# wp133716/test_isaacgym

Hardware: AMD Instinct MI355X
Metric: env-steps/sec (whole node), 4096 servo envs; 1/2/4/8-GPU scaling (higher is better)
Workload: dtype f32

## Files before the change

### test_isaacgym_amd/csrc/mg_rigid.hip

```cpp
#include "mg_internal.h"
#include "mg_math.h"
#include "mg_attractor.h"
#include "mg_contact.h"

#ifdef MG_RIGID1_STAMPS
#define MG_RIGID1_NSTAMP 18
__device__ unsigned long long g_rigid_stamp[4096][MG_RIGID1_NSTAMP];
extern "C" int mg_debug_rigid_stamps(unsigned long long* out, int nwaves) {
    if (nwaves > 4096) nwaves = 4096;
    return hipMemcpyFromSymbol(out, HIP_SYMBOL(g_rigid_stamp), (size_t)nwaves * MG_RIGID1_NSTAMP * 8) == hipSuccess
               ? 0
               : -1;
}
__device__ __forceinline__ unsigned long long rigid_stamp() {
    unsigned long long t;
    __builtin_amdgcn_sched_barrier(0);
    asm volatile("s_memtime %0\n\ts_waitcnt lgkmcnt(0)" : "=s"(t)::"memory");
    __builtin_amdgcn_sched_barrier(0);
    return t;
}
#define RSTAMP(k) do { const unsigned long long t_ = rigid_stamp(); \
    if (threadIdx.x == 0 && blockIdx.x < 4096) g_rigid_stamp[blockIdx.x][k] = t_; } while (0)
#define RUSE(v) asm volatile("" ::"v"(v))
#else
#define RSTAMP(k) do { } while (0)
#define RUSE(v) do { } while (0)
#endif

namespace {

__device__ __forceinline__ float fdot3(V3 a, V3 b, float acc) {
    return fmaf(a.z, b.z, fmaf(a.y, b.y, fmaf(a.x, b.x, acc)));
}
__device__ __forceinline__ V3 fmad3(V3 v, V3 d, float s) {
    return v3(fmaf(d.x, s, v.x), fmaf(d.y, s, v.y), fmaf(d.z, s, v.z));
}
struct BasisGen {
    static constexpr bool kPacked = false;
    V3 n, t1, t2;
    __device__ __forceinline__ float dn(V3 v) const { return vdot(n, v); }
    __device__ __forceinline__ float d1(V3 v) const { return vdot(t1, v); }
    __device__ __forceinline__ float d2(V3 v) const { return vdot(t2, v); }
    __device__ __forceinline__ V3 cn(V3 r) const { return vcross(r, n); }
    __device__ __forceinline__ V3 c1(V3 r) const { return vcross(r, t1); }
    __device__ __forceinline__ V3 c2(V3 r) const { return vcross(r, t2); }
    __device__ __forceinline__ V3 addn(V3 v, float s) const { return vmad(v, n, s); }
    __device__ __forceinline__ V3 add1(V3 v, float s) const { return vmad(v, t1, s); }
    __device__ __forceinline__ V3 add2(V3 v, float s) const { return vmad(v, t2, s); }
    __device__ __forceinline__ float vn(V3 v, V3 w, V3 r) const { return fdot3(w, cn(r), vdot(n, v)); }
    __device__ __forceinline__ float v1(V3 v, V3 w, V3 r) const { return fdot3(w, c1(r), vdot(t1, v)); }
    __device__ __forceinline__ float v2(V3 v, V3 w, V3 r) const { return fdot3(w, c2(r), vdot(t2, v)); }
    __device__ __forceinline__ float ps(float s0, V3 dx, V3 dth, V3 r) const {
        return fdot3(dth, cn(r), s0 + vdot(n, dx));
    }
    __device__ __forceinline__ V3 fn(V3 v, float dl, float invm) const { return fmad3(v, n, dl * invm); }
    __device__ __forceinline__ V3 f1(V3 v, float dl, float invm) const { return fmad3(v, t1, dl * invm); }
    __device__ __forceinline__ V3 f2(V3 v, float dl, float invm) const { return fmad3(v, t2, dl * invm); }
    __device__ __forceinline__ V3 iwn(const S3& I, V3 r) const { return symmul(I, cn(r)); }
    __device__ __forceinline__ V3 iw1(const S3& I, V3 r) const { return symmul(I, c1(r)); }
    __device__ __forceinline__ V3 iw2(const S3& I, V3 r) const { return symmul(I, c2(r)); }
    __device__ __forceinline__ float kn(V3 r, V3 In) const { return vdot(cn(r), In); }
    __device__ __forceinline__ float k1(V3 r, V3 I1) const { return vdot(c1(r), I1); }
    __device__ __forceinline__ float k2(V3 r, V3 I2) const { return vdot(c2(r), I2); }
};
struct BasisZ {
    static constexpr bool kPacked = true;
    __device__ __forceinline__ float dn(V3 v) const { return v.z; }
    __device__ __forceinline__ float d1(V3 v) const { return v.y; }
    __device__ __forceinline__ float d2(V3 v) const { return -v.x; }
    __device__ __forceinline__ V3 cn(V3 r) const { return v3(r.y, -r.x, 0.0f); }
    __device__ __forceinline__ V3 c1(V3 r) const { return v3(-r.z, 0.0f, r.x); }
    __device__ __forceinline__ V3 c2(V3 r) const { return v3(0.0f, -r.z, r.y); }
    __device__ __forceinline__ V3 addn(V3 v, float s) const { return v3(v.x, v.y, v.z + s); }
    __device__ __forceinline__ V3 add1(V3 v, float s) const { return v3(v.x, v.y + s, v.z); }
    __device__ __forceinline__ V3 add2(V3 v, float s) const { return v3(v.x - s, v.y, v.z); }
    __device__ __forceinline__ float vn(V3 v, V3 w, V3 r) const { return fmaf(w.y, -r.x, fmaf(w.x, r.y, v.z)); }
    __device__ __forceinline__ float v1(V3 v, V3 w, V3 r) const { return fmaf(w.z, r.x, fmaf(w.x, -r.z, v.y)); }
    __device__ __forceinline__ float v2(V3 v, V3 w, V3 r) const { return fmaf(w.z, r.y, fmaf(w.y, -r.z, -v.x)); }
    __device__ __forceinline__ float ps(float s0, V3 dx, V3 dth, V3 r) const {
        return fmaf(dth.y, -r.x, fmaf(dth.x, r.y, s0 + dx.z));
    }
    __device__ __forceinline__ V3 fn(V3 v, float dl, float invm) const { return v3(v.x, v.y, fmaf(dl, invm, v.z)); }
    __device__ __forceinline__ V3 f1(V3 v, float dl, float invm) const { return v3(v.x, fmaf(dl, invm, v.y), v.z); }
    __device__ __forceinline__ V3 f2(V3 v, float dl, float invm) const { return v3(fmaf(-dl, invm, v.x), v.y, v.z); }
    __device__ __forceinline__ V3 iwn(const S3& I, V3 r) const {
        const float a = r.y, b = -r.x;
        return v3(I.xx * a + I.xy * b, I.xy * a + I.yy * b, I.xz * a + I.yz * b);
    }
    __device__ __forceinline__ V3 iw1(const S3& I, V3 r) const {
        const float a = -r.z, c = r.x;
        return v3(I.xx * a + I.xz * c, I.xy * a + I.yz * c, I.xz * a + I.zz * c);
    }
    __device__ __forceinline__ V3 iw2(const S3& I, V3 r) const {
        const float b = -r.z, c = r.y;
        return v3(I.xy * b + I.xz * c, I.yy * b + I.yz * c, I.yz * b + I.zz * c);
    }
    __device__ __forceinline__ float kn(V3 r, V3 In) const { return r.y * In.x + -r.x * In.y; }
    __device__ __forceinline__ float k1(V3 r, V3 I1) const { return -r.z * I1.x + r.x * I1.z; }
    __device__ __forceinline__ float k2(V3 r, V3 I2) const { return -r.z * I2.y + r.y * I2.z; }
};

__device__ __forceinline__ float clamp_sym(float x, float lim) { return __builtin_amdgcn_fmed3f(x, -lim, lim); }

struct Slot {
    V3 r;
    float s0;
    float mu, e;
    float kn, kt1, kt2;
    float ln, lt1, lt2;
    float vn0;
    V3 In, I1, I2;
    bool on;
};

#define MG_OPAQUE3(v) asm volatile("" : "+v"((v).x), "+v"((v).y), "+v"((v).z))

template <bool CACHE, class B>
__device__ __forceinline__ void contact_normal(const B& G, Slot& c, V3& v, V3& w, float invm, const S3& Iw,
                                               float tgt) {
    if (!CACHE) MG_OPAQUE3(c.r);
    const float vn = G.vn(v, w, c.r);
    const float nl = fmaxf(fmaf(c.kn, tgt - vn, c.ln), 0.0f);
    const float dl = nl - c.ln;
    c.ln = nl;
    v = G.fn(v, dl, invm);
    w = fmad3(w, CACHE ? c.In : G.iwn(Iw, c.r), dl);
}

template <bool CACHE, class B>
__device__ __forceinline__ void contact_friction(const B& G, Slot& c, V3& v, V3& w, float invm, const S3& Iw) {
    if (!CACHE) MG_OPAQUE3(c.r);
    const float lim = c.mu * c.ln;
    const float vt1 = G.v1(v, w, c.r);
    const float n1 = clamp_sym(fmaf(-c.kt1, vt1, c.lt1), lim);
    const float d1 = n1 - c.lt1;
    c.lt1 = n1;
    v = G.f1(v, d1, invm);
    w = fmad3(w, CACHE ? c.I1 : G.iw1(Iw, c.r), d1);
    const float vt2 = G.v2(v, w, c.r);
    const float n2 = clamp_sym(fmaf(-c.kt2, vt2, c.lt2), lim);
    const float d2 = n2 - c.lt2;
    c.lt2 = n2;
    v = G.f2(v, d2, invm);
    w = fmad3(w, CACHE ? c.I2 : G.iw2(Iw, c.r), d2);
}

__device__ __forceinline__ float pos_target(const MgStep& P, float s) { return fminf(-s * P.inv_sub, P.max_depen); }
__device__ __forceinline__ float vel_target(const MgStep& P, float s, float e, float vn0) {
    float tgt = fminf(-s * P.inv_h, 0.0f);
    if (e > 0.0f && vn0 < -P.bounce_thresh) tgt = fmaxf(tgt, -e * vn0);
    return tgt;
}

__device__ __forceinline__ bool shape_pose_identity(const float* sh) {
    return sh[4] == 0.0f && sh[5] == 0.0f && sh[6] == 0.0f && sh[7] == 0.0f && sh[8] == 0.0f && sh[9] == 0.0f &&
           sh[10] == 1.0f;
}
__device__ __forceinline__ Q4 inertia_frame(Q4 q, Q4 iq) {
    if (iq.x == 0.0f && iq.y == 0.0f && iq.z == 0.0f && iq.w == 1.0f) return q;
    return qmul(q, iq);
}
__device__ __forceinline__ V3 com_world(V3 x, Q4 q, V3 com) {
    if (com.x == 0.0f && com.y == 0.0f && com.z == 0.0f) return x;
    return vadd(x, qrot(q, com));
}
__device__ __forceinline__ V3 origin_from_com(V3 xc, Q4 q, V3 com) {
    if (com.x == 0.0f && com.y == 0.0f && com.z == 0.0f) return xc;
    return vsub(xc, qrot(q, com));
}

template <bool BOX = false, class B, class F>
__device__ __forceinline__ void shape_candidates(const B& G, const MgStep& P, const float* sh, Q4 q, V3 x,
                                                 const float* hulls, F&& emit) {
    const int type = BOX ? MG_SHAPE_BOX : (int)sh[0];
    Q4 qs = q;
    V3 cs = x;
    if constexpr (!BOX) {
        if (!shape_pose_identity(sh)) {
            qs = qmul(q, q4(sh[7], sh[8], sh[9], sh[10]));
            cs = vadd(x, qrot(q, v3(sh[4], sh[5], sh[6])));
        }
    }
    const float mu = 0.5f * (sh[11] + P.mu_ground);
    const float e = 0.5f * (sh[12] + P.e_ground);
    if (type == MG_SHAPE_BOX) {
        const M3 Rs = qmat(qs);
        const float d0 = G.dn(Rs.c0), d1 = G.dn(Rs.c1), d2 = G.dn(Rs.c2);
        const float ad0 = fabsf(d0), ad1 = fabsf(d1), ad2 = fabsf(d2);
        int ia = 0;
        float best = ad0;
        if (ad1 > best) { ia = 1; best = ad1; }
        if (ad2 > best) ia = 2;
        const V3 a0 = vscale(Rs.c0, sh[1]);
        const V3 a1 = vscale(Rs.c1, sh[2]);
        const V3 a2 = vscale(Rs.c2, sh[3]);
        const float di = ia == 0 ? d0 : (ia == 1 ? d1 : d2);
        const V3 ai = ia == 0 ? a0 : (ia == 1 ? a1 : a2);
        const V3 e1 = ia == 0 ? a1 : a0;
        const V3 e2 = ia == 2 ? a1 : a2;
        const V3 u = vscale(ai, di > 0.0f ? -1.0f : 1.0f);
        const V3 cu = vadd(cs, u);
#pragma unroll
        for (int k = 0; k < 4; ++k) {
            const float sx = (k & 1) ? 1.0f : -1.0f;
            const float sy = (k & 2) ? 1.0f : -1.0f;
            const V3 p = vadd(vadd(cu, vscale(e1, sx)), vscale(e2, sy));
            emit(k, p, G.dn(p) + P.pd, mu, e);
        }
    } else if (type == MG_SHAPE_SPHERE) {
        const float rad = sh[1];
        emit(0, G.addn(cs, -rad), G.dn(cs) + P.pd - rad, mu, e);
    } else if (type == MG_SHAPE_CAPSULE) {
        const float rad = sh[1];
        const V3 ax = vscale(qrot(qs, v3(1.0f, 0.0f, 0.0f)), sh[2]);
#pragma unroll
        for (int k = 0; k < 2; ++k) {
            const V3 c = k ? vadd(cs, ax) : vsub(cs, ax);
            emit(k, G.addn(c, -rad), G.dn(c) + P.pd - rad, mu, e);
        }
    } else if (type == MG_SHAPE_CONVEX) {
        const float* hv = hulls + (int)sh[2];
        const int nv = (int)hv[0];
        float ks[4] = {0.0f, 0.0f, 0.0f, 0.0f};
        V3 kp[4];
        int kn = 0;
        for (int i = 0; i < nv; ++i) {
            const float* v = hv + MG_HULL_HEADER + 3 * i;
            const V3 p = vadd(cs, qrot(qs, v3(v[0], v[1], v[2])));
            const float sep = G.dn(p) + P.pd;
            if (!(sep < P.contact_offset)) continue;
            if (kn == 4 && !(sep < ks[3])) continue;
            int at = 0;
#pragma unroll
            for (int k = 0; k < 4; ++k)
                if (k < kn && ks[k] <= sep) at = k + 1;
#pragma unroll
            for (int k = 3; k > 0; --k)
                if (k > at) { ks[k] = ks[k - 1]; kp[k] = kp[k - 1]; }
#pragma unroll
            for (int k = 0; k < 4; ++k)
                if (k == at) { ks[k] = sep; kp[k] = p; }
            if (kn < 4) kn = kn + 1;
        }
#pragma unroll
        for (int k = 0; k < 4; ++k)
            if (k < kn) emit(k, kp[k], ks[k], mu, e);
    }
}

template <int MAXC, bool MULTI, bool ATTR, bool CREP, class B>
__device__ __forceinline__ void rigid_body(const B& G, const MgStep& P, const MgRigidArgs& A, int b) {
    constexpr bool CACHE = !MULTI;
    const int nb = A.nb;
    float* S = A.state;

    V3 x = v3(S[0 * nb + b], S[1 * nb + b], S[2 * nb + b]);
    Q4 q = q4(S[3 * nb + b], S[4 * nb + b], S[5 * nb + b], S[6 * nb + b]);
    V3 v = v3(S[7 * nb + b], S[8 * nb + b], S[9 * nb + b]);
    V3 w = v3(S[10 * nb + b], S[11 * nb + b], S[12 * nb + b]);

    const float* M = A.mass;
    const float invm = M[0 * nb + b];
    const V3 invI = v3(M[1 * nb + b], M[2 * nb + b], M[3 * nb + b]);
    const Q4 iq = q4(M[4 * nb + b], M[5 * nb + b], M[6 * nb + b], M[7 * nb + b]);
    const V3 com = v3(M[8 * nb + b], M[9 * nb + b], M[10 * nb + b]);

    const int tb = A.body_tmpl[b];
    const float lin_damp = A.tbf[tb * MG_TBODY_F_N + 0];
    const float ang_damp = A.tbf[tb * MG_TBODY_F_N + 1];
    const float max_lv = A.tbf[tb * MG_TBODY_F_N + 2];
    const float max_av = A.tbf[tb * MG_TBODY_F_N + 3];
    const float grav_on = A.tbf[tb * MG_TBODY_F_N + 4];
    const int sh0 = A.tbi[tb * MG_TBODY_I_N + 0];
    const int nsh = A.tbi[tb * MG_TBODY_I_N + 1];

    V3 fext = v3(0.0f, 0.0f, 0.0f), text = v3(0.0f, 0.0f, 0.0f);
    if (A.ext) {
        fext = v3(A.ext[0 * nb + b], A.ext[1 * nb + b], A.ext[2 * nb + b]);
        text = v3(A.ext[3 * nb + b], A.ext[4 * nb + b], A.ext[5 * nb + b]);
    }

    const float h = P.h;
    const float lin_keep = 1.0f - fminf(lin_damp * h, 1.0f);
    const float ang_keep = 1.0f - fminf(ang_damp * h, 1.0f);
    const float max_lv2 = max_lv * max_lv;
    const float max_av2 = max_av * max_av;
    const float* at = nullptr;
    if constexpr (ATTR) {
        const int ai = A.attr_idx[b];
        if (ai >= 0) at = A.attr + (size_t)ai * MG_ATTR_N;
    }

    q = qnormalize(q);
    V3 fsum = v3(0.0f, 0.0f, 0.0f);
    int crk = 0;

    for (int st = 0; st < P.substeps; ++st) {
        const S3 Iw = sym_rdrt(qmat(inertia_frame(q, iq)), invI);
        const V3 xc = com_world(x, q, com);

        if (grav_on != 0.0f) v = vmad(v, v3(P.g[0], P.g[1], P.g[2]), h);
        if (A.ext) {
            v = vmad(v, fext, invm * h);
            w = vmad(w, symmul(Iw, text), h);
        }
        if constexpr (ATTR) {
            if (at) attr_free_body(at, x, q, xc, invm, invI, iq, h, v, w);
        }
        v = vscale(v, lin_keep);
        w = vscale(w, ang_keep);
        {
            float v2 = vdot(v, v);
            if (v2 > max_lv2) v = vscale(v, sqrtf(max_lv2 / v2));
            float w2 = vdot(w, w);
            if (w2 > max_av2) w = vscale(w, sqrtf(max_av2 / w2));
        }

        Slot sl[MAXC];
#pragma unroll
        for (int j = 0; j < MAXC; ++j) sl[j].on = false;
        if (P.has_ground) {
            if constexpr (!MULTI) {
                if (nsh == 1)
                shape_candidates(G, P, A.shapes + sh0 * MG_SHAPE_STRIDE, q, x, A.hulls,
                                 [&](int k, V3 p, float sep, float mu, float e) {
                                     if (sep < P.contact_offset) {
                                         sl[k].on = true;
                                         sl[k].r = vsub(p, xc);
                                         sl[k].s0 = sep - P.rest_offset;
                                         sl[k].mu = mu;
                                         sl[k].e = e;
                                     }
                                 });
            } else {
                int nc = 0;
                for (int s = sh0; s < sh0 + nsh; ++s) {
                    shape_candidates(G, P, A.shapes + s * MG_SHAPE_STRIDE, q, x, A.hulls,
                                     [&](int, V3 p, float sep, float mu, float e) {
                                         if (sep < P.contact_offset && nc < MAXC) {
#pragma unroll
                                             for (int j = MAXC - 1; j > 0; --j) {
                                                 sl[j].r = sl[j - 1].r; sl[j].s0 = sl[j - 1].s0;
                                                 sl[j].mu = sl[j - 1].mu; sl[j].e = sl[j - 1].e;
                                                 sl[j].on = sl[j - 1].on;
                                             }
                                             sl[0].r = vsub(p, xc); sl[0].s0 = sep - P.rest_offset;
                                             sl[0].mu = mu; sl[0].e = e; sl[0].on = true;
                                             nc = nc + 1;
                                         }
                                     });
                }
            }
        }
#pragma unroll
        for (int j = 0; j < MAXC; ++j) {
            if (sl[j].on) {
                const V3 In = G.iwn(Iw, sl[j].r), I1 = G.iw1(Iw, sl[j].r), I2 = G.iw2(Iw, sl[j].r);
                if (CACHE) { sl[j].In = In; sl[j].I1 = I1; sl[j].I2 = I2; }
                sl[j].kn = 1.0f / (invm + G.kn(sl[j].r, In));
                sl[j].kt1 = 1.0f / (invm + G.k1(sl[j].r, I1));
                sl[j].kt2 = 1.0f / (invm + G.k2(sl[j].r, I2));
                sl[j].ln = 0.0f; sl[j].lt1 = 0.0f; sl[j].lt2 = 0.0f;
                sl[j].vn0 = G.vn(v, w, sl[j].r);
            }
        }

        V3 dx = v3(0.0f, 0.0f, 0.0f), dth = v3(0.0f, 0.0f, 0.0f);
        for (int it = 0; it < P.npos; ++it) {
#pragma unroll
            for (int j = 0; j < MAXC; ++j) {
                if (sl[j].on) {
                    const float s = G.ps(sl[j].s0, dx, dth, sl[j].r);
                    contact_normal<CACHE>(G, sl[j], v, w, invm, Iw, pos_target(P, s));
                }
            }
#pragma unroll
            for (int j = 0; j < MAXC; ++j)
                if (sl[j].on) contact_friction<CACHE>(G, sl[j], v, w, invm, Iw);
            dx = fmad3(dx, v, P.sub);
            dth = fmad3(dth, w, P.sub);
        }
        for (int it = 0; it < P.nvel; ++it) {
#pragma unroll
            for (int j = 0; j < MAXC; ++j) {
                if (sl[j].on) {
                    const float s = G.ps(sl[j].s0, dx, dth, sl[j].r);
                    contact_normal<CACHE>(G, sl[j], v, w, invm, Iw, vel_target(P, s, sl[j].e, sl[j].vn0));
                }
            }
#pragma unroll
            for (int j = 0; j < MAXC; ++j)
                if (sl[j].on) contact_friction<CACHE>(G, sl[j], v, w, invm, Iw);
        }
#pragma unroll
        for (int j = 0; j < MAXC; ++j) {
            if (sl[j].on) {
                fsum = G.addn(fsum, sl[j].ln);
                fsum = G.add1(fsum, sl[j].lt1);
                fsum = G.add2(fsum, sl[j].lt2);
            }
        }
        if constexpr (CREP) {
            if (st == P.substeps - 1) {
                const V3 z3 = v3(0.0f, 0.0f, 0.0f);
                const int gb = A.crep_body[b];
#pragma unroll
                for (int j = 0; j < MAXC; ++j) {
                    if (sl[j].on && crk < MG_CREP_FREE_CAP) {
                        crep_store(A.crep + b, A.crep_stride, crk, gb, -1, 0, vadd(xc, sl[j].r), G.addn(z3, 1.0f),
                                   sl[j].s0, sl[j].ln, G.add2(G.add1(z3, sl[j].lt1), sl[j].lt2), sl[j].mu);
                        crk = crk + 1;
                    }
                }
            }
        }

        const V3 xc1 = vadd(xc, dx);
        q = qintegrate(q, dth);
        x = origin_from_com(xc1, q, com);
    }

    S[0 * nb + b] = x.x; S[1 * nb + b] = x.y; S[2 * nb + b] = x.z;
    S[3 * nb + b] = q.x; S[4 * nb + b] = q.y; S[5 * nb + b] = q.z; S[6 * nb + b] = q.w;
    S[7 * nb + b] = v.x; S[8 * nb + b] = v.y; S[9 * nb + b] = v.z;
    S[10 * nb + b] = w.x; S[11 * nb + b] = w.y; S[12 * nb + b] = w.z;
    A.cforce[0 * nb + b] = fsum.x * P.inv_dt;
    A.cforce[1 * nb + b] = fsum.y * P.inv_dt;
    A.cforce[2 * nb + b] = fsum.z * P.inv_dt;
    if constexpr (CREP) A.crep_n[b] = crk;
}

#ifndef MG_RIGID1_SHAPE_REGS
#define MG_RIGID1_SHAPE_REGS 1
#endif
struct GPatch {
    int cnt;
    bool dirty;
    V3 nA;
    V3 aA[2];
    V3 aB[2];
};
template <class B>
__device__ __forceinline__ void ground_patch_update(const B& G, GPatch& R, V3 x, Q4 q, V3 n0, const V3 (&p)[4],
                                                    const float (&s0)[4], const bool (&on)[4], float fot,
                                                    float corr) {
    const float c2 = corr * corr;
    const V3 z3 = v3(0.0f, 0.0f, 0.0f);
    int cnt = R.cnt;
    const float nd = G.dn(qrot(q, R.nA));
    if (cnt > 0 && nd < MG_FP_NORMAL_COS) cnt = 0;
    const V3 wa0 = vadd(x, qrot(q, R.aA[0]));
    const V3 wa1 = vadd(x, qrot(q, R.aA[1]));
    const V3 d0v = vsub(wa0, R.aB[0]), d1v = vsub(wa1, R.aB[1]);
    const bool k0 = 0 < cnt && vdot(d0v, d0v) <= c2;
    const bool k1 = 1 < cnt && vdot(d1v, d1v) <= c2;
    GPatch N;
    N.aA[0] = vsel(k0, R.aA[0], vsel(k1, R.aA[1], z3));
    N.aB[0] = vsel(k0, R.aB[0], vsel(k1, R.aB[1], z3));
    N.aA[1] = vsel(k0 && k1, R.aA[1], z3);
    N.aB[1] = vsel(k0 && k1, R.aB[1], z3);
    V3 w0 = vsel(k0, wa0, vsel(k1, wa1, z3));
    V3 w1 = z3;
    const int kept = (k0 ? 1 : 0) + (k1 ? 1 : 0);
    int nc = kept;
    float dd = 0.0f;
    bool set0 = false, set1 = false;
#pragma unroll
    for (int j = 0; j < 4; ++j) {
        const bool c = kept < 2 && on[j] && s0[j] <= fot;
        const V3 pj = p[j];
        const V3 e0 = vsub(pj, w0), e1 = vsub(pj, w1);
        const float dj0 = vdot(e0, e0), dj1 = vdot(e1, e1);
        const bool a0 = c && nc == 0;
        const bool a1 = c && nc == 1 && dj0 > c2;
        const bool a2 = c && nc == 2 && dj0 > dj1 && dj0 > dd;
        const bool a3 = c && nc == 2 && !(dj0 > dj1) && dj1 > dd;
        const bool to0 = a0 || a3, to1 = a1 || a2;
        dd = (a1 || a2) ? dj0 : (a3 ? dj1 : dd);
        w0 = vsel(to0, pj, w0);
        w1 = vsel(to1, pj, w1);
        set0 = set0 || to0;
        set1 = set1 || to1;
        nc = a0 ? 1 : (a1 ? 2 : nc);
    }
    N.aA[0] = vsel(set0, qrot_inv(q, vsub(w0, x)), N.aA[0]);
    N.aB[0] = vsel(set0, w0, N.aB[0]);
    N.aA[1] = vsel(set1, qrot_inv(q, vsub(w1, x)), N.aA[1]);
    N.aB[1] = vsel(set1, w1, N.aB[1]);
    N.cnt = nc;
    N.nA = vsel(kept > 0, R.nA, qrot_inv(q, n0));
    N.dirty = R.dirty || !(kept == R.cnt && nc == kept);
    R = N;
}

struct NRow {
    V3 r, In;
    float s0, kn, ln, vn0;
};
struct ARow {
    V3 r, I1, I2;
    float k1, k2, l1, l2;
    float e1, e2;
};

template <class B>
__device__ __forceinline__ void row_normal1(const B& G, NRow& c, V3& v, V3& w, float invm, float tgt) {
    const float vn = G.vn(v, w, c.r);
    const float nl = fmaxf(fmaf(c.kn, tgt - vn, c.ln), 0.0f);
    const float dl = nl - c.ln;
    c.ln = nl;
    v = G.fn(v, dl, invm);
    w = fmad3(w, c.In, dl);
}

typedef float f2 __attribute__((ext_vector_type(2)));
__device__ __forceinline__ f2 pk2(float a, float b) { return f2{a, b}; }
__device__ __forceinline__ f2 bc2(float a) { return f2{a, a}; }
__device__ __forceinline__ f2 pfma(f2 a, f2 b, f2 c) { return __builtin_elementwise_fma(a, b, c); }

__device__ __forceinline__ void tgs_zp(const MgStep& P, NRow (&sl)[4], ARow (&an)[2], float lim1, float e, V3& v,
                                       V3& w, V3& dx, V3& dth, float invm, bool& c01, bool& c02, bool& c11,
                                       bool& c12) {
    f2 W = pk2(w.x, w.y), Z = pk2(w.z, v.z), V = pk2(v.x, v.y);
    f2 DW = pk2(dth.x, dth.y), DZ = pk2(dth.z, dx.z), DV = pk2(dx.x, dx.y);
    float s0r[4];
#pragma unroll
    for (int j = 0; j < 4; ++j) {
        s0r[j] = sl[j].s0;
        asm volatile("" : "+v"(s0r[j]));
    }
    const f2 S0a = pk2(s0r[0], s0r[1]), S0b = pk2(s0r[2], s0r[3]);
    const f2 RYa = pk2(sl[0].r.y, sl[1].r.y), RYb = pk2(sl[2].r.y, sl[3].r.y);
    const f2 NRXa = pk2(-sl[0].r.x, -sl[1].r.x), NRXb = pk2(-sl[2].r.x, -sl[3].r.x);
    auto sep = [&](int h) {
        f2 a = (h ? S0b : S0a) + bc2(DZ.y);
        a = pfma(bc2(DW.x), h ? RYb : RYa, a);
        return pfma(bc2(DW.y), h ? NRXb : NRXa, a);
    };
    auto normal = [&](int j, float tgt) {
        const float nrx = -sl[j].r.x, ry = sl[j].r.y;
        const float vn = fmaf(W.y, nrx, fmaf(W.x, ry, Z.y));
        const float nl = fmaxf(fmaf(sl[j].kn, tgt - vn, sl[j].ln), 0.0f);
        const float dl = nl - sl[j].ln;
        sl[j].ln = nl;
        W = pfma(pk2(sl[j].In.x, sl[j].In.y), bc2(dl), W);
        Z = pfma(pk2(sl[j].In.z, invm), bc2(dl), Z);
    };
    auto anchors = [&](bool pos, bool last) {
        const float lim = lim1 * (((sl[0].ln + sl[1].ln) + sl[2].ln) + sl[3].ln);
#pragma unroll
        for (int a = 0; a < 2; ++a) {
            const float rx = an[a].r.x, ry = an[a].r.y, nrz = -an[a].r.z;
            {
                const float v1 = fmaf(Z.x, rx, fmaf(W.x, nrz, V.y));
                const float raw = fmaf(an[a].k1, (pos ? an[a].e1 : 0.0f) - v1, an[a].l1);
                const float nl = clamp_sym(raw, lim);
                const float dl = nl - an[a].l1;
                const bool cl = last && (raw > lim || raw < -lim);
                if (a == 0) c01 = cl; else c11 = cl;
                an[a].l1 = nl;
                V.y = fmaf(dl, invm, V.y);
                W = pfma(pk2(an[a].I1.x, an[a].I1.y), bc2(dl), W);
                Z.x = fmaf(an[a].I1.z, dl, Z.x);
            }
            {
                const float v2 = fmaf(Z.x, ry, fmaf(W.y, nrz, -V.x));
                const float raw = fmaf(an[a].k2, (pos ? an[a].e2 : 0.0f) - v2, an[a].l2);
                const float nl = clamp_sym(raw, lim);
                const float dl = nl - an[a].l2;
                const bool cl = last && (raw > lim || raw < -lim);
                if (a == 0) c02 = cl; else c12 = cl;
                an[a].l2 = nl;
                V.x = fmaf(-dl, invm, V.x);
                W = pfma(pk2(an[a].I2.x, an[a].I2.y), bc2(dl), W);
                Z.x = fmaf(an[a].I2.z, dl, Z.x);
            }
        }
    };
    const f2 nsub = bc2(-P.inv_sub), psub = bc2(P.sub);
    const int nit = P.npos + P.nvel;
    for (int it = 0; it < P.npos; ++it) {
        const f2 t0 = sep(0) * nsub, t1 = sep(1) * nsub;
        const float tg[4] = {fminf(t0.x, P.max_depen), fminf(t0.y, P.max_depen), fminf(t1.x, P.max_depen),
                             fminf(t1.y, P.max_depen)};
        if (it == 0) {
#pragma unroll
            for (int j = 0; j < 4; ++j) normal(j, tg[j]);
        }
        anchors(true, it == nit - 1);
#pragma unroll
        for (int j = 0; j < 4; ++j) normal(j, tg[j]);
        DV = pfma(V, psub, DV);
        DW = pfma(W, psub, DW);
        DZ = pfma(Z, psub, DZ);
    }
    if (P.nvel > 0) {
        const f2 s01 = sep(0), s23 = sep(1);
        const float sj[4] = {s01.x, s01.y, s23.x, s23.y};
        float tg[4];
#pragma unroll
        for (int j = 0; j < 4; ++j) tg[j] = vel_target(P, sj[j], e, sl[j].vn0);
        for (int it = P.npos; it < nit; ++it) {
#pragma unroll
            for (int j = 0; j < 4; ++j) normal(j, tg[j]);
            anchors(false, it == nit - 1);
#pragma unroll
            for (int j = 0; j < 4; ++j) normal(j, tg[j]);
        }
    }
    v = v3(V.x, V.y, Z.y);
    w = v3(W.x, W.y, Z.x);
    dx = v3(DV.x, DV.y, DZ.y);
    dth = v3(DW.x, DW.y, DZ.x);
}

template <bool PACK, bool ATTR, bool CREP, bool BOX = false, class B>
__device__ __forceinline__ int rigid_body1(const B& G, const MgStep& P, const float* T, V3& x, Q4& q, V3& v,
                                           V3& w, V3& fsum, float invm, V3 invI, Q4 iq, V3 com, bool has_ext,
                                           V3 fext, V3 text, const float* hulls, float* gp, int gstride,
                                           const float (&pr)[MG_FP_N], const float* at, float* cr = nullptr,
                                           int crs = 0, int gbody = 0) {
    int crk = 0;
    const float lin_damp = T[0], ang_damp = T[1], max_lv = T[2], max_av = T[3], grav_on = T[4];
    float shr[MG_SHAPE_STRIDE];
    const float* sh = T + MG_TBODY_F_N;
    if constexpr (PACK && MG_RIGID1_SHAPE_REGS) {
#pragma unroll
        for (int k = 0; k < 14; ++k) shr[k] = sh[k];
        sh = shr;
    }
    const bool has_shape = P.has_ground && sh[0] >= 0.0f;
    const float rho = sh[13];
    const float h = P.h;
    const float lin_keep = 1.0f - fminf(lin_damp * h, 1.0f);
    const float ang_keep = 1.0f - fminf(ang_damp * h, 1.0f);
    const float max_lv2 = max_lv * max_lv;
    const float max_av2 = max_av * max_av;
    const float mu = 0.5f * (sh[11] + P.mu_ground);
    const float e = 0.5f * (sh[12] + P.e_ground);
    const V3 n0 = v3(P.n[0], P.n[1], P.n[2]);
    GPatch R;
    R.cnt = 0;
    R.dirty = false;
    R.nA = R.aA[0] = R.aA[1] = R.aB[0] = R.aB[1] = v3(0.0f, 0.0f, 0.0f);
    {
        const float clear = G.dn(x) + P.pd;
        const bool far = rho >= 0.0f && clear - rho > P.contact_offset + 1e-3f * (1.0f + fabsf(clear) + rho);
        const bool use = gp && has_shape && !far;
        if constexpr (PACK) {
            R.cnt = (int)(use ? pr[0] : 0.0f);
            R.nA = vsel(use, v3(pr[1], pr[2], pr[3]), R.nA);
#pragma unroll
            for (int k = 0; k < 2; ++k) {
                R.aA[k] = vsel(use, v3(pr[4 + 6 * k], pr[5 + 6 * k], pr[6 + 6 * k]), R.aA[k]);
                R.aB[k] = vsel(use, v3(pr[7 + 6 * k], pr[8 + 6 * k], pr[9 + 6 * k]), R.aB[k]);
            }
        } else if (use) {
            float r[MG_FP_N];
#pragma unroll
            for (int k = 0; k < MG_FP_N; ++k) r[k] = gp[(size_t)k * gstride];
            R.cnt = (int)r[0];
            R.nA = v3(r[1], r[2], r[3]);
#pragma unroll
            for (int k = 0; k < 2; ++k) {
                R.aA[k] = v3(r[4 + 6 * k], r[5 + 6 * k], r[6 + 6 * k]);
                R.aB[k] = v3(r[7 + 6 * k], r[8 + 6 * k], r[9 + 6 * k]);
            }
        }
    }

    RUSE(R.cnt); RUSE(R.aA[1].z);
    RSTAMP(2);
    q = qnormalize(q);
    for (int st = 0; st < P.substeps; ++st) {
        const S3 Iw = sym_rdrt(qmat(inertia_frame(q, iq)), invI);
        const V3 xc = com_world(x, q, com);

        if (grav_on != 0.0f) v = vmad(v, v3(P.g[0], P.g[1], P.g[2]), h);
        if (has_ext) {
            v = vmad(v, fext, invm * h);
            w = vmad(w, symmul(Iw, text), h);
        }
        if constexpr (ATTR) {
            if (at) attr_free_body(at, x, q, xc, invm, invI, iq, h, v, w);
        }
        v = vscale(v, lin_keep);
        w = vscale(w, ang_keep);
        {
            float v2 = vdot(v, v);
            if (v2 > max_lv2) v = vscale(v, sqrtf(max_lv2 / v2));
            float w2 = vdot(w, w);
            if (w2 > max_av2) w = vscale(w, sqrtf(max_av2 / w2));
        }

        RUSE(v.x); RUSE(w.z); RUSE(xc.x);
        if (st < 2) RSTAMP(3 + 6 * st);
        NRow sl[4];
        bool on[4];
        V3 cp[4];
#pragma unroll
        for (int j = 0; j < 4; ++j) {
            on[j] = false;
            sl[j].r = v3(0.0f, 0.0f, 0.0f);
            sl[j].s0 = 0.0f;
            cp[j] = v3(0.0f, 0.0f, 0.0f);
        }
        const float clear = G.dn(x) + P.pd;
        const bool far = rho >= 0.0f && clear - rho > P.contact_offset + 1e-3f * (1.0f + fabsf(clear) + rho);
        if (__any(has_shape && !far) && has_shape)
            shape_candidates<BOX>(G, P, sh, q, x, hulls, [&](int k, V3 p, float sep, float, float) {
                const bool c = sep < P.contact_offset;
                on[k] = on[k] || c;
                sl[k].r = vsel(c, vsub(p, xc), sl[k].r);
                sl[k].s0 = c ? sep - P.rest_offset : sl[k].s0;
                cp[k] = vsel(c, p, cp[k]);
            });
        RUSE(sl[0].s0); RUSE(sl[3].r.z);
        if (st < 2) RSTAMP(4 + 6 * st);
        bool any = false;
#pragma unroll
        for (int j = 0; j < 4; ++j) any = any || on[j];
        if (any) {
            float cs0[4];
#pragma unroll
            for (int j = 0; j < 4; ++j) cs0[j] = sl[j].s0;
            ground_patch_update(G, R, x, q, n0, cp, cs0, on, P.fric_offset, P.fric_corr);
        } else {
            R.cnt = 0;
        }

        RUSE(R.cnt);
        if (st < 2) RSTAMP(5 + 6 * st);
        V3 dx = v3(0.0f, 0.0f, 0.0f), dth = v3(0.0f, 0.0f, 0.0f);
        if (__any(any)) {
#pragma unroll
            for (int j = 0; j < 4; ++j) {
                sl[j].In = G.iwn(Iw, sl[j].r);
                sl[j].kn = on[j] ? 1.0f / (invm + G.kn(sl[j].r, sl[j].In)) : 0.0f;
                sl[j].ln = 0.0f;
                sl[j].vn0 = G.vn(v, w, sl[j].r);
            }
            ARow an[2];
            V3 awp[2];
#pragma unroll
            for (int a = 0; a < 2; ++a) {
                const bool act = a < R.cnt;
                const V3 wa = vadd(x, qrot(q, R.aA[a]));
                if constexpr (CREP) awp[a] = wa;
                const V3 dr = vsub(wa, R.aB[a]);
                const float kd = 0.8f * P.inv_h;
                const V3 r = vsel(act, vsub(wa, xc), v3(0.0f, 0.0f, 0.0f));
                const float e1 = act ? fminf(fmaxf(-G.d1(dr) * kd, -P.max_depen), P.max_depen) : 0.0f;
                const float e2 = act ? fminf(fmaxf(-G.d2(dr) * kd, -P.max_depen), P.max_depen) : 0.0f;
                an[a].r = r;
                an[a].I1 = G.iw1(Iw, r);
                an[a].I2 = G.iw2(Iw, r);
                an[a].k1 = act ? 1.0f / (invm + G.k1(r, an[a].I1)) : 0.0f;
                an[a].k2 = act ? 1.0f / (invm + G.k2(r, an[a].I2)) : 0.0f;
                an[a].l1 = 0.0f;
                an[a].l2 = 0.0f;
                an[a].e1 = e1;
                an[a].e2 = e2;
            }
            bool c01 = false, c02 = false, c11 = false, c12 = false;
            const float share = R.cnt == 2 ? 0.5f : 1.0f;
            const int nit = P.npos + P.nvel;
            RUSE(an[1].k2); RUSE(sl[3].kn);
            if (st < 2) RSTAMP(6 + 6 * st);
            if constexpr (B::kPacked && PACK) {
                tgs_zp(P, sl, an, share * mu, e, v, w, dx, dth, invm, c01, c02, c11, c12);
            } else
            for (int it = 0; it < nit; ++it) {
                const bool pos = it < P.npos, last = it == nit - 1;
                auto normals = [&]() {
#pragma unroll
                    for (int j = 0; j < 4; ++j) {
                        const float sj = G.ps(sl[j].s0, dx, dth, sl[j].r);
                        row_normal1(G, sl[j], v, w, invm, pos ? pos_target(P, sj) : vel_target(P, sj, e, sl[j].vn0));
                    }
                };
                if (it == 0 || !pos) normals();
                const float mun = mu * (((sl[0].ln + sl[1].ln) + sl[2].ln) + sl[3].ln);
#pragma unroll
                for (int a = 0; a < 2; ++a) {
                    {
                        const float lim = share * mun;
                        const float raw = fmaf(an[a].k1, (pos ? an[a].e1 : 0.0f) - G.v1(v, w, an[a].r), an[a].l1);
                        const float nl = clamp_sym(raw, lim);
                        const float dl = nl - an[a].l1;
                        const bool cl = last && (raw > lim || raw < -lim);
                        if (a == 0) c01 = cl; else c11 = cl;
                        an[a].l1 = nl;
                        v = G.f1(v, dl, invm);
                        w = fmad3(w, an[a].I1, dl);
                    }
                    {
                        const float lim = share * mun;
                        const float raw = fmaf(an[a].k2, (pos ? an[a].e2 : 0.0f) - G.v2(v, w, an[a].r), an[a].l2);
                        const float nl = clamp_sym(raw, lim);
                        const float dl = nl - an[a].l2;
                        const bool cl = last && (raw > lim || raw < -lim);
                        if (a == 0) c02 = cl; else c12 = cl;
                        an[a].l2 = nl;
                        v = G.f2(v, dl, invm);
                        w = fmad3(w, an[a].I2, dl);
                    }
                }
                normals();
                if (pos) {
                    dx = fmad3(dx, v, P.sub);
                    dth = fmad3(dth, w, P.sub);
                }
            }
#pragma unroll
            for (int j = 0; j < 4; ++j) fsum = G.addn(fsum, sl[j].ln);
#pragma unroll
            for (int a = 0; a < 2; ++a) {
                fsum = G.add1(fsum, an[a].l1);
                fsum = G.add2(fsum, an[a].l2);
            }
            if constexpr (CREP) {
                if (cr && st == P.substeps - 1) {
                    const V3 z3 = v3(0.0f, 0.0f, 0.0f);
#pragma unroll
                    for (int j = 0; j < 4; ++j) {
                        if (on[j]) {
                            crep_store(cr, crs, crk, gbody, -1, 0, cp[j], n0, sl[j].s0, sl[j].ln, z3, mu);
                            crk = crk + 1;
                        }
                    }
#pragma unroll
                    for (int a = 0; a < 2; ++a) {
                        if (a < R.cnt) {
                            crep_store(cr, crs, crk, gbody, -1, 1, awp[a], n0, 0.0f, 0.0f,
                                       G.add2(G.add1(z3, an[a].l1), an[a].l2), mu);
                            crk = crk + 1;
                        }
                    }
                }
            }
            const bool one = R.cnt < 2;
            if ((c01 && (c11 || one)) || (c02 && (c12 || one))) R.cnt = 0;
        } else {
            for (int it = 0; it < P.npos; ++it) {
                dx = fmad3(dx, v, P.sub);
                dth = fmad3(dth, w, P.sub);
            }
        }

        RUSE(dx.x); RUSE(dth.z);
        if (st < 2) RSTAMP(7 + 6 * st);
        const V3 xc1 = vadd(xc, dx);
        q = qintegrate(q, dth);
        x = origin_from_com(xc1, q, com);
        RUSE(x.x); RUSE(q.w);
        if (st < 2) RSTAMP(8 + 6 * st);
    }
    if (gp && has_shape) {
        gp[0] = (float)R.cnt;
        if (R.cnt > 0 && R.dirty) {
            const float r[MG_FP_N] = {0.0f, R.nA.x, R.nA.y, R.nA.z,
                                      R.aA[0].x, R.aA[0].y, R.aA[0].z, R.aB[0].x, R.aB[0].y, R.aB[0].z,
                                      R.aA[1].x, R.aA[1].y, R.aA[1].z, R.aB[1].x, R.aB[1].y, R.aB[1].z};
#pragma unroll
            for (int k = 1; k < MG_FP_N; ++k) gp[(size_t)k * gstride] = r[k];
        }
    }
    return crk;
}

#ifndef MG_RIGID1_ROUND_WAVES
#define MG_RIGID1_ROUND_WAVES 2
#endif
#ifndef MG_RIGID1_WIDE_WAVES
#define MG_RIGID1_WIDE_WAVES 3
#endif
template <bool UPZ, bool LDS_T, bool WIDE, bool ATTR, bool REC = false, bool CREP = false, bool BOX = false>
__global__ void __launch_bounds__(64, UPZ && WIDE && !CREP ? MG_RIGID1_WIDE_WAVES : (UPZ ? MG_RIGID1_ROUND_WAVES : 2))
k_rigid_step1(MgStep P, MgRigidArgs A) {
    static_assert(!BOX || (!WIDE && REC), "BOX: a one-round build that reads the slot record");
    extern __shared__ float s_trec[];
    const int i = (WIDE ? gridDim.x - 1 - blockIdx.x : blockIdx.x) * 64 + threadIdx.x;
    RSTAMP(0);
    if constexpr (!WIDE) {
        asm volatile("" ::"s"(A.nf), "s"(A.free_ids), "s"(A.nb), "s"(A.slot_rec), "s"(A.gpatch), "s"(A.gstride),
                     "s"(A.trec), "s"(A.ntb), "s"(A.ext), "s"(A.root_src), "s"(A.state), "s"(P.h));
    }
    const bool live = i < A.nf;
    const int b = A.free_ids ? A.free_ids[live ? i : A.nf - 1] : (live ? i : A.nf - 1);
    const int nb = A.nb;
    V3 x, v, w;
    Q4 q;
    int tb;
    V3 fext = v3(0.0f, 0.0f, 0.0f), text = v3(0.0f, 0.0f, 0.0f);
    const float* T;
    int pre_ob = -1, pre_or = -1;
    float pr[MG_FP_N];
    if constexpr (WIDE) {
        const float* Si = A.state + b;
        int si = nb;
        if (A.root_src) {
            const int rr = A.root_row[b];
            if (rr >= 0) {
                Si = A.root_src + (size_t)rr * MG_STATE_N;
                si = 1;
            }
        }
        x = v3(Si[0 * si], Si[1 * si], Si[2 * si]);
        q = q4(Si[3 * si], Si[4 * si], Si[5 * si], Si[6 * si]);
        v = v3(Si[7 * si], Si[8 * si], Si[9 * si]);
        w = v3(Si[10 * si], Si[11 * si], Si[12 * si]);
        tb = A.body_tmpl[b];
        if (A.ext) {
            fext = v3(A.ext[0 * nb + b], A.ext[1 * nb + b], A.ext[2 * nb + b]);
            text = v3(A.ext[3 * nb + b], A.ext[4 * nb + b], A.ext[5 * nb + b]);
// ... 305 lines not shown
```

Baseline: 298.8 million.

## Pack rigid-body contact geometry math into paired f2 vector ops

New measurement: 306.4 million (median of 6 runs). +2.5%, better.

```diff
diff --git a/test_isaacgym_amd/csrc/mg_pair.h b/test_isaacgym_amd/csrc/mg_pair.h
--- /dev/null
+++ b/test_isaacgym_amd/csrc/mg_pair.h
@@ -0,0 +1,100 @@
+#pragma once
+#include "mg_math.h"
+
+typedef float f2 __attribute__((ext_vector_type(2)));
+MG_HD f2 pk2(float a, float b) { return f2{a, b}; }
+MG_HD f2 bc2(float a) { return f2{a, a}; }
+MG_HD f2 pfma(f2 a, f2 b, f2 c) { return __builtin_elementwise_fma(a, b, c); }
+
+struct V3x2 { f2 x, y, z; };
+struct Q4x2 { f2 x, y, z, w; };
+
+MG_HD V3x2 v3x2(V3 a, V3 b) { V3x2 r; r.x = pk2(a.x, b.x); r.y = pk2(a.y, b.y); r.z = pk2(a.z, b.z); return r; }
+MG_HD V3x2 v3bc(V3 a) { return v3x2(a, a); }
+MG_HD V3x2 v3p(f2 x, f2 y, f2 z) { V3x2 r; r.x = x; r.y = y; r.z = z; return r; }
+MG_HD V3 v3lo(V3x2 p) { return v3(p.x.x, p.y.x, p.z.x); }
+MG_HD V3 v3hi(V3x2 p) { return v3(p.x.y, p.y.y, p.z.y); }
+MG_HD Q4x2 q4x2(Q4 a, Q4 b) {
+    Q4x2 r; r.x = pk2(a.x, b.x); r.y = pk2(a.y, b.y); r.z = pk2(a.z, b.z); r.w = pk2(a.w, b.w); return r;
+}
+MG_HD Q4 q4lo(Q4x2 p) { return q4(p.x.x, p.y.x, p.z.x, p.w.x); }
+MG_HD Q4 q4hi(Q4x2 p) { return q4(p.x.y, p.y.y, p.z.y, p.w.y); }
+
+MG_HD V3x2 vadd2(V3x2 a, V3x2 b) { return v3p(a.x + b.x, a.y + b.y, a.z + b.z); }
+MG_HD V3x2 vsub2(V3x2 a, V3x2 b) { return v3p(a.x - b.x, a.y - b.y, a.z - b.z); }
+MG_HD V3x2 vscale2(V3x2 a, f2 s) { return v3p(a.x * s, a.y * s, a.z * s); }
+MG_HD f2 vdot2(V3x2 a, V3x2 b) { return a.x * b.x + a.y * b.y + a.z * b.z; }
+MG_HD V3x2 vcross2(V3x2 a, V3x2 b) {
+    return v3p(a.y * b.z - a.z * b.y, a.z * b.x - a.x * b.z, a.x * b.y - a.y * b.x);
+}
+MG_HD V3x2 vmad2(V3x2 a, V3x2 b, f2 s) { return v3p(a.x + b.x * s, a.y + b.y * s, a.z + b.z * s); }
+
+MG_HD V3x2 qrotq2(Q4x2 q, V3x2 v) {
+    const f2 tx = 2.0f * (q.y * v.z - q.z * v.y);
+    const f2 ty = 2.0f * (q.z * v.x - q.x * v.z);
+    const f2 tz = 2.0f * (q.x * v.y - q.y * v.x);
+    return v3p(v.x + q.w * tx + (q.y * tz - q.z * ty),
+               v.y + q.w * ty + (q.z * tx - q.x * tz),
+               v.z + q.w * tz + (q.x * ty - q.y * tx));
+}
+MG_HD V3x2 qrot2(Q4 q, V3x2 v) { return qrotq2(q4x2(q, q), v); }
+MG_HD V3x2 qrot_inv2(Q4 q, V3x2 v) { return qrot2(qconj(q), v); }
+
+MG_HD V3 z_iwn(const S3& I, V3 r) {
+    const float a = r.y, b = -r.x;
+    return v3(I.xx * a + I.xy * b, I.xy * a + I.yy * b, I.xz * a + I.yz * b);
+}
+MG_HD V3 z_iw1(const S3& I, V3 r) {
+    const float a = -r.z, c = r.x;
+    return v3(I.xx * a + I.xz * c, I.xy * a + I.yz * c, I.xz * a + I.zz * c);
+}
+MG_HD V3 z_iw2(const S3& I, V3 r) {
+    const float b = -r.z, c = r.y;
+    return v3(I.xy * b + I.xz * c, I.yy * b + I.yz * c, I.yz * b + I.zz * c);
+}
+MG_HD float z_kn(V3 r, V3 In) { return r.y * In.x + -r.x * In.y; }
+MG_HD float z_k1(V3 r, V3 I1) { return -r.z * I1.x + r.x * I1.z; }
+MG_HD float z_k2(V3 r, V3 I2) { return -r.z * I2.y + r.y * I2.z; }
+MG_HD V3x2 z_iwn2(const S3& I, V3x2 r) {
+    const f2 a = r.y, b = -r.x;
+    return v3p(I.xx * a + I.xy * b, I.xy * a + I.yy * b, I.xz * a + I.yz * b);
+}
+MG_HD V3x2 z_iw12(const S3& I, V3x2 r) {
+    const f2 a = -r.z, c = r.x;
+    return v3p(I.xx * a + I.xz * c, I.xy * a + I.yz * c, I.xz * a + I.zz * c);
+}
+MG_HD V3x2 z_iw22(const S3& I, V3x2 r) {
+    const f2 b = -r.z, c = r.y;
+    return v3p(I.xy * b + I.xz * c, I.yy * b + I.yz * c, I.yz * b + I.zz * c);
+}
+MG_HD f2 z_kn2(V3x2 r, V3x2 In) { return r.y * In.x + -r.x * In.y; }
+MG_HD f2 z_k12(V3x2 r, V3x2 I1) { return -r.z * I1.x + r.x * I1.z; }
+MG_HD f2 z_k22(V3x2 r, V3x2 I2) { return -r.z * I2.y + r.y * I2.z; }
+
+struct S3P { f2 xx_xy, xy_yy, xz_yz; };
+MG_HD S3P s3p(const S3& I) { S3P p; p.xx_xy = pk2(I.xx, I.xy); p.xy_yy = pk2(I.xy, I.yy); p.xz_yz = pk2(I.xz, I.yz); return p; }
+MG_HD S3 sym_rdrt_p(M3 Rp, V3 d, S3P& Ip) {
+    const f2 c0 = pk2(Rp.c0.x, Rp.c0.y), c1 = pk2(Rp.c1.x, Rp.c1.y), c2 = pk2(Rp.c2.x, Rp.c2.y);
+    const f2 u0 = c0 * bc2(d.x), u1 = c1 * bc2(d.y), u2 = c2 * bc2(d.z);
+    const float u0z = Rp.c0.z * d.x, u1z = Rp.c1.z * d.y, u2z = Rp.c2.z * d.z;
+    const f2 xx_xy = bc2(u0.x) * c0 + bc2(u1.x) * c1 + bc2(u2.x) * c2;
+    const f2 xz_yz = u0 * bc2(Rp.c0.z) + u1 * bc2(Rp.c1.z) + u2 * bc2(Rp.c2.z);
+    S3 s;
+    s.xx = xx_xy.x;
+    s.xy = xx_xy.y;
+    s.xz = xz_yz.x;
+    s.yz = xz_yz.y;
+    s.yy = u0.y * Rp.c0.y + u1.y * Rp.c1.y + u2.y * Rp.c2.y;
+    s.zz = u0z * Rp.c0.z + u1z * Rp.c1.z + u2z * Rp.c2.z;
+    Ip.xx_xy = xx_xy;
+    Ip.xy_yy = pk2(s.xy, s.yy);
+    Ip.xz_yz = xz_yz;
+    return s;
+}
+MG_HD f2 z_iwn_xy(const S3P& I, V3 r) { return I.xx_xy * bc2(r.y) + I.xy_yy * bc2(-r.x); }
+MG_HD f2 z_iw1_xy(const S3P& I, V3 r) { return I.xx_xy * bc2(-r.z) + I.xz_yz * bc2(r.x); }
+MG_HD f2 z_iw2_xy(const S3P& I, V3 r) { return I.xy_yy * bc2(-r.z) + I.xz_yz * bc2(r.y); }
+MG_HD float z_iwn_z(const S3& I, V3 r) { return I.xz * r.y + I.yz * -r.x; }
+MG_HD float z_iw1_z(const S3& I, V3 r) { return I.xz * -r.z + I.zz * r.x; }
+MG_HD float z_iw2_z(const S3& I, V3 r) { return I.yz * -r.z + I.zz * r.y; }
+MG_HD f2 z_vn2(V3 v, V3 w, f2 ry, f2 nrx) { return pfma(bc2(w.y), nrx, pfma(bc2(w.x), ry, bc2(v.z))); }
diff --git a/test_isaacgym_amd/csrc/mg_rigid.hip b/test_isaacgym_amd/csrc/mg_rigid.hip
--- a/test_isaacgym_amd/csrc/mg_rigid.hip
+++ b/test_isaacgym_amd/csrc/mg_rigid.hip
@@ -1,5 +1,6 @@
 #include "mg_internal.h"
 #include "mg_math.h"
+#include "mg_pair.h"
 #include "mg_attractor.h"
 #include "mg_contact.h"
 
@@ -83,21 +84,12 @@
     __device__ __forceinline__ V3 fn(V3 v, float dl, float invm) const { return v3(v.x, v.y, fmaf(dl, invm, v.z)); }
     __device__ __forceinline__ V3 f1(V3 v, float dl, float invm) const { return v3(v.x, fmaf(dl, invm, v.y), v.z); }
     __device__ __forceinline__ V3 f2(V3 v, float dl, float invm) const { return v3(fmaf(-dl, invm, v.x), v.y, v.z); }
-    __device__ __forceinline__ V3 iwn(const S3& I, V3 r) const {
-        const float a = r.y, b = -r.x;
-        return v3(I.xx * a + I.xy * b, I.xy * a + I.yy * b, I.xz * a + I.yz * b);
-    }
-    __device__ __forceinline__ V3 iw1(const S3& I, V3 r) const {
-        const float a = -r.z, c = r.x;
-        return v3(I.xx * a + I.xz * c, I.xy * a + I.yz * c, I.xz * a + I.zz * c);
-    }
-    __device__ __forceinline__ V3 iw2(const S3& I, V3 r) const {
-        const float b = -r.z, c = r.y;
-        return v3(I.xy * b + I.xz * c, I.yy * b + I.yz * c, I.yz * b + I.zz * c);
-    }
-    __device__ __forceinline__ float kn(V3 r, V3 In) const { return r.y * In.x + -r.x * In.y; }
-    __device__ __forceinline__ float k1(V3 r, V3 I1) const { return -r.z * I1.x + r.x * I1.z; }
-    __device__ __forceinline__ float k2(V3 r, V3 I2) const { return -r.z * I2.y + r.y * I2.z; }
+    __device__ __forceinline__ V3 iwn(const S3& I, V3 r) const { return z_iwn(I, r); }
+    __device__ __forceinline__ V3 iw1(const S3& I, V3 r) const { return z_iw1(I, r); }
+    __device__ __forceinline__ V3 iw2(const S3& I, V3 r) const { return z_iw2(I, r); }
+    __device__ __forceinline__ float kn(V3 r, V3 In) const { return z_kn(r, In); }
+    __device__ __forceinline__ float k1(V3 r, V3 I1) const { return z_k1(r, I1); }
+    __device__ __forceinline__ float k2(V3 r, V3 I2) const { return z_k2(r, I2); }
 };
 
 __device__ __forceinline__ float clamp_sym(float x, float lim) { return __builtin_amdgcn_fmed3f(x, -lim, lim); }
@@ -169,9 +161,9 @@
     return vsub(xc, qrot(q, com));
 }
 
-template <bool BOX = false, class B, class F>
+template <bool BOX = false, bool PK = false, class B, class F>
 __device__ __forceinline__ void shape_candidates(const B& G, const MgStep& P, const float* sh, Q4 q, V3 x,
-                                                 const float* hulls, F&& emit) {
+                                                 const float* hulls, F&& emit, const M3* Rq = nullptr) {
     const int type = BOX ? MG_SHAPE_BOX : (int)sh[0];
     Q4 qs = q;
     V3 cs = x;
@@ -184,7 +176,15 @@
     const float mu = 0.5f * (sh[11] + P.mu_ground);
     const float e = 0.5f * (sh[12] + P.e_ground);
     if (type == MG_SHAPE_BOX) {
-        const M3 Rs = qmat(qs);
+        M3 Rs;
+        if constexpr (PK) {
+            Rs = *Rq;
+            if constexpr (!BOX) {
+                if (!shape_pose_identity(sh)) Rs = qmat(qs);
+            }
+        } else {
+            Rs = qmat(qs);
+        }
         const float d0 = G.dn(Rs.c0), d1 = G.dn(Rs.c1), d2 = G.dn(Rs.c2);
         const float ad0 = fabsf(d0), ad1 = fabsf(d1), ad2 = fabsf(d2);
         int ia = 0;
@@ -432,6 +432,9 @@
 
 #ifndef MG_RIGID1_SHAPE_REGS
 #define MG_RIGID1_SHAPE_REGS 1
+#endif
+#ifndef MG_RIGID1_PACK_GEOM
+#define MG_RIGID1_PACK_GEOM 1
 #endif
 struct GPatch {
     int cnt;
@@ -493,6 +496,64 @@
     R = N;
 }
 
+template <class B>
+__device__ __forceinline__ void ground_patch_update_pk(const B& G, GPatch& R, V3 x, Q4 q, V3 n0, const V3 (&p)[4],
+                                                       const float (&s0)[4], const bool (&on)[4], float fot,
+                                                       float corr) {
+    const float c2 = corr * corr;
+    const V3 z3 = v3(0.0f, 0.0f, 0.0f);
+    int cnt = R.cnt;
+    const V3x2 nn = qrotq2(q4x2(q, qconj(q)), v3x2(R.nA, n0));
+    const float nd = G.dn(v3lo(nn));
+    if (cnt > 0 && nd < MG_FP_NORMAL_COS) cnt = 0;
+    const V3x2 X = v3bc(x);
+    const V3x2 wa = vadd2(X, qrot2(q, v3x2(R.aA[0], R.aA[1])));
+    const V3x2 dv = vsub2(wa, v3x2(R.aB[0], R.aB[1]));
+    const f2 dq = vdot2(dv, dv);
+    const bool k0 = 0 < cnt && dq.x <= c2;
+    const bool k1 = 1 < cnt && dq.y <= c2;
+    const V3 wa0 = v3lo(wa), wa1 = v3hi(wa);
+    GPatch N;
+    N.aA[0] = vsel(k0, R.aA[0], vsel(k1, R.aA[1], z3));
+    N.aB[0] = vsel(k0, R.aB[0], vsel(k1, R.aB[1], z3));
+    N.aA[1] = vsel(k0 && k1, R.aA[1], z3);
+    N.aB[1] = vsel(k0 && k1, R.aB[1], z3);
+    V3x2 W = v3x2(vsel(k0, wa0, vsel(k1, wa1, z3)), z3);
+    const int kept = (k0 ? 1 : 0) + (k1 ? 1 : 0);
+    int nc = kept;
+    float dd = 0.0f;
+    bool set0 = false, set1 = false;
+#pragma unroll
+    for (int j = 0; j < 4; ++j) {
+        const bool c = kept < 2 && on[j] && s0[j] <= fot;
+        const V3 pj = p[j];
+        const V3x2 E = vsub2(v3bc(pj), W);
+        const f2 dj = vdot2(E, E);
+        const float dj0 = dj.x, dj1 = dj.y;
+        const bool a0 = c && nc == 0;
+        const bool a1 = c && nc == 1 && dj0 > c2;
+        const bool a2 = c && nc == 2 && dj0 > dj1 && dj0 > dd;
+        const bool a3 = c && nc == 2 && !(dj0 > dj1) && dj1 > dd;
+        const bool to0 = a0 || a3, to1 = a1 || a2;
+        dd = (a1 || a2) ? dj0 : (a3 ? dj1 : dd);
+        W.x = pk2(to0 ? pj.x : W.x.x, to1 ? pj.x : W.x.y);
+        W.y = pk2(to0 ? pj.y : W.y.x, to1 ? pj.y : W.y.y);
+        W.z = pk2(to0 ? pj.z : W.z.x, to1 ? pj.z : W.z.y);
+        set0 = set0 || to0;
+        set1 = set1 || to1;
+        nc = a0 ? 1 : (a1 ? 2 : nc);
+    }
+    const V3x2 bA = qrot_inv2(q, vsub2(W, X));
+    N.aA[0] = vsel(set0, v3lo(bA), N.aA[0]);
+    N.aB[0] = vsel(set0, v3lo(W), N.aB[0]);
+    N.aA[1] = vsel(set1, v3hi(bA), N.aA[1]);
+    N.aB[1] = vsel(set1, v3hi(W), N.aB[1]);
+    N.cnt = nc;
+    N.nA = vsel(kept > 0, R.nA, v3hi(nn));
+    N.dirty = R.dirty || !(kept == R.cnt && nc == kept);
+    R = N;
+}
+
 struct NRow {
     V3 r, In;
     float s0, kn, ln, vn0;
@@ -513,10 +574,6 @@
     w = fmad3(w, c.In, dl);
 }
 
-typedef float f2 __attribute__((ext_vector_type(2)));
-__device__ __forceinline__ f2 pk2(float a, float b) { return f2{a, b}; }
-__device__ __forceinline__ f2 bc2(float a) { return f2{a, a}; }
-__device__ __forceinline__ f2 pfma(f2 a, f2 b, f2 c) { return __builtin_elementwise_fma(a, b, c); }
 
 __device__ __forceinline__ void tgs_zp(const MgStep& P, NRow (&sl)[4], ARow (&an)[2], float lim1, float e, V3& v,
                                        V3& w, V3& dx, V3& dth, float invm, bool& c01, bool& c02, bool& c11,
@@ -621,6 +678,7 @@
                                            const float (&pr)[MG_FP_N], const float* at, float* cr = nullptr,
                                            int crs = 0, int gbody = 0) {
     int crk = 0;
+    constexpr bool PKG = PACK && !ATTR && !CREP && MG_RIGID1_PACK_GEOM;
     const float lin_damp = T[0], ang_damp = T[1], max_lv = T[2], max_av = T[3], grav_on = T[4];
     float shr[MG_SHAPE_STRIDE];
     const float* sh = T + MG_TBODY_F_N;
@@ -673,7 +731,17 @@
     RSTAMP(2);
     q = qnormalize(q);
     for (int st = 0; st < P.substeps; ++st) {
-        const S3 Iw = sym_rdrt(qmat(inertia_frame(q, iq)), invI);
+        M3 Rq;
+        S3P Ip;
+        S3 Iw;
+        if constexpr (PKG) {
+            Rq = qmat(q);
+            M3 Rp = Rq;
+            if (!(iq.x == 0.0f && iq.y == 0.0f && iq.z == 0.0f && iq.w == 1.0f)) Rp = qmat(qmul(q, iq));
+            Iw = sym_rdrt_p(Rp, invI, Ip);
+        } else {
+            Iw = sym_rdrt(qmat(inertia_frame(q, iq)), invI);
+        }
         const V3 xc = com_world(x, q, com);
 
         if (grav_on != 0.0f) v = vmad(v, v3(P.g[0], P.g[1], P.g[2]), h);
@@ -708,13 +776,13 @@
         const float clear = G.dn(x) + P.pd;
         const bool far = rho >= 0.0f && clear - rho > P.contact_offset + 1e-3f * (1.0f + fabsf(clear) + rho);
         if (__any(has_shape && !far) && has_shape)
-            shape_candidates<BOX>(G, P, sh, q, x, hulls, [&](int k, V3 p, float sep, float, float) {
+            shape_candidates<BOX, PKG>(G, P, sh, q, x, hulls, [&](int k, V3 p, float sep, float, float) {
                 const bool c = sep < P.contact_offset;
                 on[k] = on[k] || c;
                 sl[k].r = vsel(c, vsub(p, xc), sl[k].r);
                 sl[k].s0 = c ? sep - P.rest_offset : sl[k].s0;
                 cp[k] = vsel(c, p, cp[k]);
-            });
+            }, &Rq);
         RUSE(sl[0].s0); RUSE(sl[3].r.z);
         if (st < 2) RSTAMP(4 + 6 * st);
         bool any = false;
@@ -724,7 +792,10 @@
             float cs0[4];
 #pragma unroll
             for (int j = 0; j < 4; ++j) cs0[j] = sl[j].s0;
-            ground_patch_update(G, R, x, q, n0, cp, cs0, on, P.fric_offset, P.fric_corr);
+            if constexpr (PKG)
+                ground_patch_update_pk(G, R, x, q, n0, cp, cs0, on, P.fric_offset, P.fric_corr);
+            else
+                ground_patch_update(G, R, x, q, n0, cp, cs0, on, P.fric_offset, P.fric_corr);
         } else {
             R.cnt = 0;
         }
@@ -733,34 +804,70 @@
         if (st < 2) RSTAMP(5 + 6 * st);
         V3 dx = v3(0.0f, 0.0f, 0.0f), dth = v3(0.0f, 0.0f, 0.0f);
         if (__any(any)) {
-#pragma unroll
-            for (int j = 0; j < 4; ++j) {
-                sl[j].In = G.iwn(Iw, sl[j].r);
-                sl[j].kn = on[j] ? 1.0f / (invm + G.kn(sl[j].r, sl[j].In)) : 0.0f;
-                sl[j].ln = 0.0f;
-                sl[j].vn0 = G.vn(v, w, sl[j].r);
-            }
             ARow an[2];
             V3 awp[2];
-#pragma unroll
-            for (int a = 0; a < 2; ++a) {
-                const bool act = a < R.cnt;
-                const V3 wa = vadd(x, qrot(q, R.aA[a]));
-                if constexpr (CREP) awp[a] = wa;
-                const V3 dr = vsub(wa, R.aB[a]);
-                const float kd = 0.8f * P.inv_h;
-                const V3 r = vsel(act, vsub(wa, xc), v3(0.0f, 0.0f, 0.0f));
-                const float e1 = act ? fminf(fmaxf(-G.d1(dr) * kd, -P.max_depen), P.max_depen) : 0.0f;
-                const float e2 = act ? fminf(fmaxf(-G.d2(dr) * kd, -P.max_depen), P.max_depen) : 0.0f;
-                an[a].r = r;
-                an[a].I1 = G.iw1(Iw, r);
-                an[a].I2 = G.iw2(Iw, r);
-                an[a].k1 = act ? 1.0f / (invm + G.k1(r, an[a].I1)) : 0.0f;
-                an[a].k2 = act ? 1.0f / (invm + G.k2(r, an[a].I2)) : 0.0f;
-                an[a].l1 = 0.0f;
-                an[a].l2 = 0.0f;
-                an[a].e1 = e1;
-                an[a].e2 = e2;
+            if constexpr (PKG && B::kPacked) {
+#pragma unroll
+                for (int j = 0; j < 4; ++j) {
+                    const f2 Ixy = z_iwn_xy(Ip, sl[j].r);
+                    sl[j].In = v3(Ixy.x, Ixy.y, z_iwn_z(Iw, sl[j].r));
+                    sl[j].kn = on[j] ? 1.0f / (invm + G.kn(sl[j].r, sl[j].In)) : 0.0f;
+                    sl[j].ln = 0.0f;
+                }
+#pragma unroll
+                for (int j = 0; j < 4; j += 2) {
+                    const f2 vn0 = z_vn2(v, w, pk2(sl[j].r.y, sl[j + 1].r.y), pk2(-sl[j].r.x, -sl[j + 1].r.x));
+                    sl[j].vn0 = vn0.x;
+                    sl[j + 1].vn0 = vn0.y;
+                }
+                const V3x2 WA = vadd2(v3bc(x), qrot2(q, v3x2(R.aA[0], R.aA[1])));
+                const V3x2 DR = vsub2(WA, v3x2(R.aB[0], R.aB[1]));
+                const V3x2 RR = vsub2(WA, v3bc(xc));
+                const f2 kd2 = bc2(0.8f * P.inv_h);
+                const f2 E1 = -DR.y * kd2, E2 = -(-DR.x) * kd2;
+#pragma unroll
+                for (int a = 0; a < 2; ++a) {
+                    const bool act = a < R.cnt;
+                    const V3 r = vsel(act, a ? v3hi(RR) : v3lo(RR), v3(0.0f, 0.0f, 0.0f));
+                    const f2 I1xy = z_iw1_xy(Ip, r), I2xy = z_iw2_xy(Ip, r);
+                    an[a].r = r;
+                    an[a].I1 = v3(I1xy.x, I1xy.y, z_iw1_z(Iw, r));
+                    an[a].I2 = v3(I2xy.x, I2xy.y, z_iw2_z(Iw, r));
+                    an[a].k1 = act ? 1.0f / (invm + G.k1(r, an[a].I1)) : 0.0f;
+                    an[a].k2 = act ? 1.0f / (invm + G.k2(r, an[a].I2)) : 0.0f;
+                    an[a].l1 = 0.0f;
+                    an[a].l2 = 0.0f;
+                    an[a].e1 = act ? fminf(fmaxf(a ? E1.y : E1.x, -P.max_depen), P.max_depen) : 0.0f;
+                    an[a].e2 = act ? fminf(fmaxf(a ? E2.y : E2.x, -P.max_depen), P.max_depen) : 0.0f;
+                }
+            } else {
+#pragma unroll
+                for (int j = 0; j < 4; ++j) {
+                    sl[j].In = G.iwn(Iw, sl[j].r);
+                    sl[j].kn = on[j] ? 1.0f / (invm + G.kn(sl[j].r, sl[j].In)) : 0.0f;
+                    sl[j].ln = 0.0f;
+                    sl[j].vn0 = G.vn(v, w, sl[j].r);
+                }
+#pragma unroll
+                for (int a = 0; a < 2; ++a) {
+                    const bool act = a < R.cnt;
+                    const V3 wa = vadd(x, qrot(q, R.aA[a]));
+                    if constexpr (CREP) awp[a] = wa;
+                    const V3 dr = vsub(wa, R.aB[a]);
+                    const float kd = 0.8f * P.inv_h;
+                    const V3 r = vsel(act, vsub(wa, xc), v3(0.0f, 0.0f, 0.0f));
+                    const float e1 = act ? fminf(fmaxf(-G.d1(dr) * kd, -P.max_depen), P.max_depen) : 0.0f;
+                    const float e2 = act ? fminf(fmaxf(-G.d2(dr) * kd, -P.max_depen), P.max_depen) : 0.0f;
+                    an[a].r = r;
+                    an[a].I1 = G.iw1(Iw, r);
+                    an[a].I2 = G.iw2(Iw, r);
+                    an[a].k1 = act ? 1.0f / (invm + G.k1(r, an[a].I1)) : 0.0f;
+                    an[a].k2 = act ? 1.0f / (invm + G.k2(r, an[a].I2)) : 0.0f;
+                    an[a].l1 = 0.0f;
+                    an[a].l2 = 0.0f;
+                    an[a].e1 = e1;
+                    an[a].e2 = e2;
+                }
             }
             bool c01 = false, c02 = false, c11 = false, c12 = false;
             const float share = R.cnt == 2 ? 0.5f : 1.0f;
```
